# multiplefish/VPLines-SLAM

Hardware: AMD Instinct MI355X
Metric: sliding-window BA solves/sec (10 KF, 200 pts + 80 lines, 5 iters) (higher is better)
Workload: dtype f64

## Files before the change

### vplines-slam_amd/csrc/ba_common.h

```cpp
#pragma once
#include <hip/hip_runtime.h>
#include "ba_types.h"
#include "vpl_math.h"

namespace vpl {

#ifdef VPL_STAMPS
#define VPL_STAMP(B, w, i) do { if (threadIdx.x == 0) (B).dbg[(size_t)(w) * 64 + (i)] = (long long)__builtin_readcyclecounter(); } while (0)
#else
#define VPL_STAMP(B, w, i) do {} while (0)
#endif

__device__ __forceinline__ void count_active(const DevBatch& B, int k) {
  if (B.act && threadIdx.x == 0 && B.launch < ACT_SLOTS) atomicAdd(&B.act[4 * B.launch + k], 1);
}

__device__ __forceinline__ int ordered_window(const DevBatch& B) {
  const int w = B.ord_it == 0 ? (int)blockIdx.x : B.order[(size_t)(B.ord_it & 1) * B.nW + blockIdx.x];
  return __builtin_amdgcn_readfirstlane(w);
}

__device__ __forceinline__ double wave_sum(double v) {
#pragma unroll
  for (int o = 32; o > 0; o >>= 1) v += __shfl_xor(v, o, 64);
// ... 129 lines not shown
  diag_tile_step<8>(d, m, r4, cc, ncol, pivc, bad);  diag_tile_step<9>(d, m, r4, cc, ncol, pivc, bad);
  diag_tile_step<10>(d, m, r4, cc, ncol, pivc, bad); diag_tile_step<11>(d, m, r4, cc, ncol, pivc, bad);
  diag_tile_step<12>(d, m, r4, cc, ncol, pivc, bad); diag_tile_step<13>(d, m, r4, cc, ncol, pivc, bad);
  diag_tile_step<14>(d, m, r4, cc, ncol, pivc, bad); diag_tile_step<15>(d, m, r4, cc, ncol, pivc, bad);
}


__device__ __forceinline__ bool wave_chol16(double* A, int n, int ld, double* Xinv, int lane) {
  const int r4 = lane >> 4, cc = lane & 15;
  double d[4], m[4];
#pragma unroll
  for (int v = 0; v < 4; ++v) {
    const int r = r4 + 4 * v;
    d[v] = (r < n && cc < n) ? A[r * ld + cc] : (r == cc ? 1.0 : 0.0);
    m[v] = r == cc ? 1.0 : 0.0;
  }
  double pivc = 1.0;
  bool bad = false;
  diag_tile_factor(d, m, r4, cc, 16, pivc, bad);
  if (bad) return false;
  const double sq = sqrt(pivc), isq = 1.0 / sq;
#pragma unroll
  for (int v = 0; v < 4; ++v) {
    const int r = r4 + 4 * v;
    const double ir = __shfl(isq, r, 64);
    if (r < n && cc < n) {
      A[r * ld + cc] = r > cc ? d[v] / sq : (r == cc ? sq : 0.0);
      if (Xinv) Xinv[r * ld + cc] = r >= cc ? m[v] * ir : 0.0;
    }
  }
  return true;
}

}
```

### vplines-slam_amd/csrc/ba_ctx.h

```cpp
#pragma once
#include <functional>
#include <map>
#include <string>

#include "vplines_ba.h"
#include "ba_types.h"
#include "ba_stage.h"

struct vpl_ctx {
  int device = 0;
  hipStream_t stream = nullptr;
  DevBatch B;
  std::vector<void*> allocs;
  std::vector<size_t> alloc_bytes;
  bool guards = false;
  std::string err;
  int maxW = 0, maxP = 0, maxPO = 0, maxL = 0, maxLO = 0;
  int nW = 0;
  vpl_ba_options opt;
  bool upload_open = false;
  std::vector<int> h_nP, h_nL;
  std::vector<std::vector<int>> h_lmap;
  std::vector<int> h_mg_m;
  std::vector<int> h_mg_n;
  std::vector<int> h_mg_nb;
  std::vector<int> h_passthrough;
  std::vector<vpl_prior> h_pass_priors;
  bool any_second_new = false;
  int maxPriorN = 0;
  bool prior_resident = false;
  int prior_resident_nW = 0;
  std::vector<int> layout_key;
  bool layout_valid = false;
  bool force_general = false;
  bool schur_mostly_wide = false;
  bool schur_never_wide = false;
  bool schur_wide_all = false;
  bool step_fused = true;
  size_t marg_smem = 0;
  int marg_nmax = 0;
  bool marg_small = false;
  int prior_rule = VPL_PRIOR_PIVOTED_CHOLESKY;
  hipGraphExec_t graph_exec = nullptr;
  bool use_graph = true;
  bool timing = false;
  std::map<std::string, std::pair<double, int>> ktimes;
  std::vector<std::pair<const char*, double>> ltimes;
  int* d_act = nullptr;
  std::vector<std::string> kname_store;
  bool leg_timing = false;
  hipEvent_t leg_ev[6] = {nullptr, nullptr, nullptr, nullptr, nullptr, nullptr};
  double odo_ms[3] = {0, 0, 0};
  std::function<int()> pending;
  Stage stage;
  size_t last_upload_bytes = 0;
  struct vpl_odo* odo = nullptr;
};

static void drop_graph(vpl_ctx* c) {
  if (c->graph_exec) { (void)hipGraphExecDestroy(c->graph_exec); c->graph_exec = nullptr; }
}

static int settle(vpl_ctx* c) {
  if (!c || !c->pending) return VPL_OK;
  std::function<int()> fin;
  fin.swap(c->pending);
  return fin();
}
static int finish_or_defer(vpl_ctx* c, bool async, std::function<int()> fin) {
  if (!async) return fin();
// ... 34 lines not shown
```

### vplines-slam_amd/csrc/ba_lin.h

```cpp
#pragma once
#include "ba_common.h"

namespace vpl {

typedef double v4d_lin __attribute__((ext_vector_type(4)));
constexpr int LIN_THREADS = 512;
constexpr int STG_LD = 17;
constexpr int LIN_STAGE = 8 * 32 * STG_LD;
constexpr int PRE_LDS = 62;
constexpr int LIN_HW = 720;
constexpr int PREP_NMAX = 112;
__host__ __device__ constexpr int lin_stage_doubles(int maxL) {
  const int ln = 8 * LIN_HW + 38 * maxL;
  const int pt = LIN_STAGE + 78 * 36 + NV;
  const int m = ln > pt ? ln : pt;
  return m > 4650 + 3570 ? m : 4650 + 3570;
}
constexpr int PREP_THREADS = 640;
inline size_t prep_smem(int max_prior_n) {
  const int ns = max_prior_n < PREP_NMAX ? max_prior_n : PREP_NMAX;
  return (size_t)((PREP_THREADS / 64) * 675 + ns * ns) * sizeof(double);
}
constexpr size_t PREP_SMEM = (size_t)((PREP_THREADS / 64) * 675 + PREP_NMAX * PREP_NMAX) * sizeof(double);

__device__ __forceinline__ void prep_body(const DevBatch& B, const int w, double* psm, int nstage) {
  const int tid = threadIdx.x;
  const int lane = tid & 63, wv = tid >> 6;
  const int NWV = blockDim.x >> 6;
  double* wsc = psm + wv * 675;
  double* Jl = psm + NWV * 675;
  const int n = B.pr_n[w];
  const bool fits = n > 0 && n <= nstage;
  if (fits) {
    const double* J0g = B.pr_J0 + (size_t)w * B.prS;
    for (int idx = tid; idx < n * n; idx += blockDim.x) Jl[idx] = J0g[idx];
  }
  for (int j = 1 + wv; j < NF; j += NWV) {
    DevPreint& P = B.pre[(size_t)w * NF + j];
    double* G = wsc;
    double* X = wsc + 225;
    double* Pm = wsc + 450;
    for (int k = lane; k < 225; k += 64) G[k] = P.cov[k];
    __builtin_amdgcn_wave_barrier();
    wave_chol16(G, 15, 15, X, lane);
    __builtin_amdgcn_wave_barrier();
    for (int e = lane; e < 225; e += 64) {
      const int a = e / 15, b2 = e % 15;
      double s2 = 0;
      for (int k = (a > b2 ? a : b2); k < 15; ++k) s2 += X[k * 15 + a] * X[k * 15 + b2];
      Pm[e] = s2;
    }
    __builtin_amdgcn_wave_barrier();
    wave_chol16(Pm, 15, 15, nullptr, lane);
    __builtin_amdgcn_wave_barrier();
    for (int e = lane; e < 225; e += 64) {
      const int i = e / 15, jj = e % 15;
      P.sqrt_info[e] = (jj >= i) ? Pm[jj * 15 + i] : 0.0;
    }
    __builtin_amdgcn_wave_barrier();
  }
  if (tid < NF + 1) {
    double* x = tid < NF ? B.pose + ((size_t)w * NF + tid) * 7 : B.ex + (size_t)w * 7;
    Q4 q = mat2q(qmat(qnormalized(qpose(x))));
    if (tid == 0) {
      M3 R0 = qmat(qnormalized(qpose(x)));
      V3 ypr = R2ypr(R0);
      double* g = B.gauge + (size_t)w * 4;
      g[0] = ypr.x; g[1] = x[0]; g[2] = x[1]; g[3] = x[2];
      const double* fr = B.fail_ref + (size_t)w * 13;
      if (fr[0] != 0.0) {
        M3 Rl;
        for (int k = 0; k < 9; ++k) Rl.m[k] = fr[4 + k];
        g[0] = R2ypr(Rl).x; g[1] = fr[1]; g[2] = fr[2]; g[3] = fr[3];
      }
    }
    x[3] = q.x; x[4] = q.y; x[5] = q.z; x[6] = q.w;
    double* xq = psm + 7 * tid;
    xq[0] = x[0]; xq[1] = x[1]; xq[2] = x[2]; xq[3] = q.x; xq[4] = q.y; xq[5] = q.z; xq[6] = q.w;
  }
  __syncthreads();
  const int nL = B.orth_in[w] ? 0 : B.nL[w];
  for (int l = tid; l < nL; l += blockDim.x) {
    const int s = B.ln_start[(size_t)w * B.maxL + l];
    const double* ps = psm + 7 * s;
    const double* ex = psm + 7 * NF;
    M3 Rs = qmat(qpose(ps)), ric = qmat(qpose(ex));
    V3 P{ps[0], ps[1], ps[2]}, tic{ex[0], ex[1], ex[2]};
    V3 twc = P + mul(Rs, tic);
    M3 Rwc = mul(Rs, ric);
    const double* pl = B.plk + ((size_t)w * B.maxL + l) * 6;
    Plk Lc{V3{pl[0], pl[1], pl[2]}, V3{pl[3], pl[4], pl[5]}};
    Plk Lw = plk_to_pose(Lc, Rwc, twc);
    plk_to_orth(Lw, B.orth + ((size_t)w * B.maxL + l) * 4);
  }
  for (int l = tid; l < B.nL[w]; l += blockDim.x) {
    const size_t li = (size_t)w * B.maxL + l;
    const Plk Lw = orth_to_plk(B.orth + li * 4);
    double* o = B.lw + li * 6;
    o[0] = Lw.n.x; o[1] = Lw.n.y; o[2] = Lw.n.z; o[3] = Lw.v.x; o[4] = Lw.v.y; o[5] = Lw.v.z;
  }
  if (n > 0) {
    const double* J0 = B.pr_J0 + (size_t)w * B.prS;
    double* H = B.pr_H + (size_t)w * B.prS;
    const double* Js = fits ? Jl : J0;
    if (fits) {
      const int NT = (n + 15) >> 4, NLT = NT * (NT + 1) / 2, KS = (n + 3) >> 2;
      const int m = lane & 15, kk = lane >> 4;
      for (int t = wv; t < NLT; t += NWV) {
        int ta, tb;
        tri_decode(t, ta, tb);
        const int ca = 16 * ta + m, cb = 16 * tb + m;
        v4d_lin acc = {0, 0, 0, 0};
        for (int ks = 0; ks < KS; ++ks) {
          const int k = 4 * ks + kk;
          const double av = (k < n && ca < n) ? Js[k * n + ca] : 0.0;
          const double bv = (k < n && cb < n) ? Js[k * n + cb] : 0.0;
          acc = __builtin_amdgcn_mfma_f64_16x16x4f64(av, bv, acc, 0, 0, 0);
        }
        const double vals[4] = {acc.x, acc.y, acc.z, acc.w};
#pragma unroll
        for (int v = 0; v < 4; ++v) {
          const int r = 16 * ta + kk + 4 * v, c2 = cb;
          if (r < n && c2 < n && (ta != tb || r >= c2)) {
            H[(size_t)r * n + c2] = vals[v];
            H[(size_t)c2 * n + r] = vals[v];
          }
        }
      }
    } else
    for (int idx = tid; idx < n * n; idx += blockDim.x) {
      int a = idx / n, b = idx % n;
      double s = 0;
      for (int k = 0; k < n; ++k) s += Js[(size_t)k * n + a] * Js[(size_t)k * n + b];
      H[idx] = s;
    }
    for (int c2 = tid; c2 < n; c2 += blockDim.x) {
      double s = 0;
      const double* r0g = B.pr_r0 + (size_t)w * MAXPN;
#pragma unroll 8
      for (int k = 0; k < n; ++k) s += Js[(size_t)k * n + c2] * r0g[k];
      B.pr_g0[(size_t)w * MAXPN + c2] = s;
    }
    if (tid < B.pr_nb[w]) {
      int kind = B.pr_kind[(size_t)w * MAXPB + tid], fr = B.pr_frame[(size_t)w * MAXPB + tid];
      int idx = B.pr_idx[(size_t)w * MAXPB + tid];
      int base = kind == 0 ? 15 * fr : kind == 1 ? 15 * fr + 6 : 165;
      int ls = kind == 1 ? 9 : 6;
      for (int k = 0; k < ls; ++k) B.pr_map[(size_t)w * MAXPN + idx + k] = base + k;
    }
  }
  if (tid == 0) {
    TrState t;
    t.radius = 1e4; t.mu = 1e-8; t.x_cost = 0; t.cand_cost = 0; t.model_cost_change = 0; t.x_norm = 0;
    t.step_norm = 0; t.dogleg_step_norm = 0; t.alpha = 0; t.a1 = t.a2 = t.a3 = 0; t.initial_cost = 0;
    t.iter = 0; t.status = 0; t.reuse = 0; t.step_valid = 0; t.fresh_lin = 0; t.num_successful = 0; t.num_invalid = 0;
    t.pad = 0;
    B.tr[w] = t;
  }
}
__global__ __launch_bounds__(PREP_THREADS) void k_prep(DevBatch B, int nstage) {
  extern __shared__ double psm[];
  prep_body(B, blockIdx.x, psm, nstage);
}

constexpr int HV_DOUBLES = 78 * 36;
constexpr int LIN_PART = 78 * 36 + 72 + 8;
__host__ __device__ __forceinline__ int hvi(int r, int c) {
  const int br = r / 6, bc = c / 6;
  return 36 * (br * (br + 1) / 2 + bc) + 6 * (r - 6 * br) + (c - 6 * bc);
}

inline void lin_asm_entry(int r, int c, int* out) {
  int hv = 0, im = 0;
  const int vr = cam2vis(r), vc = cam2vis(c);
  if (vr >= 0 && vc >= 0) hv = hvi(vr, vc) + 1;
  if (r < 165) {
    const int fr = r / 15, ar = r - 15 * fr, fc = c / 15, bc = c - 15 * fc;
    if (fc == fr) im = 120 * fr + ar * (ar + 1) / 2 + bc + 1;
    else if (fc == fr - 1) im = 11 * 120 + 225 * (fr - 1) + 15 * ar + bc + 1;
  }
  out[0] = hv | im << 16;
  out[1] = r | c << 8;
}

template <int MODE, int ROLE>
__device__ __forceinline__ void lin_body(const DevBatch& B, const int w, double* sm) {
  constexpr bool MARG = MODE != 0;
  constexpr bool PRIOR_ONLY = MODE == 2;
  constexpr bool DO_PTS = ROLE != 2, DO_REST = ROLE != 1;
  static_assert(ROLE == 0 || MODE == 0, "the marginalisation passes are one work-group");
  const int tid = threadIdx.x, T = LIN_THREADS;
  TrState* tr = &B.tr[w];
  if (!MARG) {
    if (tr->status != 0 || tr->fresh_lin) return;
    if (DO_REST) count_active(B, 0);
  }
  if (PRIOR_ONLY && B.mg_n[w] == 0) return;
  double* Hv = sm;
  double* gv = Hv + HV_DOUBLES;
  double* xp = gv + NV;
  double* xs = xp + 84;
  double* imuJ = xs + 99;
  double* imur = imuJ + 4500;
  const int stg_doubles = lin_stage_doubles(B.maxL);
  double* prr = imuJ + stg_doubles;
  double* prdx = prr + MAXPN;
  double* prg = prdx + MAXPN;
  double* red = prg + MAXPN;
  const int PST = B.maxP | 1;
  double* pacc = red + 18;
  double* prH = pacc + 14 * PST;
  const int PRH_N = B.prhN;
  double* plds = prH + PRH_N * (PRH_N + 1) / 2;
  int* invmap = (int*)(plds + 10 * PRE_LDS);
// ... 473 lines not shown
  VPL_STAMP(B, w, 25);
  for (int i = tid; i < 4650; i += T) imuJ[i] = 0.0;
  double sa[2][4];
#pragma unroll
  for (int q = 0; q < 2; ++q) {
    const int f = (tid >> 6) + 8 * q;
    const double* S = B.pre[(size_t)w * NF + (f < 10 ? f : 0) + 1].sqrt_info;
#pragma unroll
    for (int ks = 0; ks < 4; ++ks) {
      const int k = 4 * ks + (lane >> 4), i = lane & 15;
      sa[q][ks] = (f < 10 && i < 15 && k < 15 && k >= i) ? S[i * 15 + k] : 0.0;
    }
  }
  __syncthreads();
  if ((tid & 63) < 10 && tid < 128) {
    const int f = tid & 63, j = f + 1;
    const DevPreint& dp = *(const DevPreint*)(plds + PRE_LDS * f);
    bool act = MARG ? (j == 1 && dp.sum_dt < 10.0) : !(dp.sum_dt > 10.0);
    if (PRIOR_ONLY) act = false;
    if (tid < 64) imuact[f] = act ? 1 : 0;
    if (act) {
      PreInt p = load_preint(dp);
      if (tid < 64) {
        imu_residual_raw(p, xp + 7 * (j - 1), xs + 9 * (j - 1), xp + 7 * j, xs + 9 * j, B.opt.g_norm, imur + 15 * f);
      } else {
        ImuJac JB = imu_jacobian_raw(p, xp + 7 * (j - 1), xs + 9 * (j - 1), xp + 7 * j, xs + 9 * j, B.opt.g_norm);
        imu_jac_dense(JB, imuJ + 450 * f);
      }
    }
  }
  __syncthreads();
  VPL_STAMP(B, w, 28);
  constexpr int ASM_PER_THREAD = (NCP + LIN_THREADS - 1) / LIN_THREADS;
  int2 asmd[ASM_PER_THREAD];
#pragma unroll
  for (int u = 0; u < ASM_PER_THREAD; ++u) {
    const int e = u * T + tid;
    asmd[u] = ((const int2*)B.asm_tab)[e < NCP ? e : 0];
  }
  double* imuH = imuJ + 4650;
  {
    const int wvi = tid >> 6, m16 = lane & 15, kk = lane >> 4;
    v4d_lin cd[2] = {{0, 0, 0, 0}, {0, 0, 0, 0}};
    for (int i = tid; i < 120; i += T) imuH[i] = 0.0;
#pragma unroll
    for (int q = 0; q < 2; ++q) {
      const int f = wvi + 8 * q;
      if (f >= 10) break;
      double* J = imuJ + 450 * f;
      double* rr = imur + 15 * f;
      const bool on = imuact[f] != 0;
      v4d_lin jw[2] = {{0, 0, 0, 0}, {0, 0, 0, 0}};
#pragma unroll
      for (int ct = 0; ct < 2; ++ct) {
        const int c = 16 * ct + m16;
#pragma unroll
        for (int ks = 0; ks < 4; ++ks) {
          const int k = 4 * ks + kk;
          const double bv = k < 15 ? (c < 30 ? J[k * 30 + c] : (c == 30 ? rr[k] : 0.0)) : 0.0;
          jw[ct] = __builtin_amdgcn_mfma_f64_16x16x4f64(on ? sa[q][ks] : 0.0, bv, jw[ct], 0, 0, 0);
        }
      }
      __builtin_amdgcn_wave_barrier();
      if (on) {
#pragma unroll
        for (int ct = 0; ct < 2; ++ct) {
          const double vals[4] = {jw[ct].x, jw[ct].y, jw[ct].z, jw[ct].w};
          const int c = 16 * ct + m16;
#pragma unroll
          for (int v = 0; v < 4; ++v) {
            const int r = kk + 4 * v;
// ... 48 lines not shown
#pragma unroll
      for (int v = 0; v < 4; ++v) {
        const int i0 = kk + 4 * v, j0 = m16;
        if (i0 < 15 && j0 <= i0) imuH[120 * f + i0 * (i0 + 1) / 2 + j0] += keep[v];
      }
    }
  }
  __syncthreads();
  if (tid < 10 && imuact[tid]) {
    double s = 0;
    for (int k = 0; k < 15; ++k) s += imur[15 * tid + k] * imur[15 * tid + k];
    cost += 0.5 * s;
  }


  if (ROLE == 2) {
    if (tid == 0) {
      while (__hip_atomic_load(&B.lin_flag[w], __ATOMIC_RELAXED, __HIP_MEMORY_SCOPE_AGENT) != 1) __builtin_amdgcn_s_sleep(32);
      __hip_atomic_store(&B.lin_flag[w], 0, __ATOMIC_RELAXED, __HIP_MEMORY_SCOPE_AGENT);
    }
    __syncthreads();
    const double* part = B.lin_part + (size_t)w * LIN_PART;
    for (int i = tid; i < HV_DOUBLES + NV; i += T) sm[i] += __hip_atomic_load(&part[i], __ATOMIC_RELAXED, __HIP_MEMORY_SCOPE_AGENT);
    if (tid == 0) cost += __hip_atomic_load(&part[HV_DOUBLES + NV], __ATOMIC_RELAXED, __HIP_MEMORY_SCOPE_AGENT);
    __syncthreads();
  } else if (!MARG) {
    if (tid == 0) cost += cost_pts;
  }
  VPL_STAMP(B, w, 20);
  double* Hout = B.Hcc + (size_t)w * NCP;
  const double* pH = B.pr_H + (size_t)w * B.prS;
  VPL_STAMP(B, w, 26);
  const bool prior_lds = n > 0 && n <= PRH_N;
  {
#pragma unroll
    for (int u = 0; u < ASM_PER_THREAD; ++u) {
      const int e = u * T + tid;
      if (e >= NCP) continue;
      const int hv = asmd[u].x & 0xffff, im = asmd[u].x >> 16, r = asmd[u].y & 255, c = asmd[u].y >> 8;
      const double vh = Hv[hv ? hv - 1 : 0], vi = imuH[im ? im - 1 : 0];
      const int ir = prior_lds ? invmap[r] : -1, ic = prior_lds ? invmap[c] : -1;
      const bool hp = ir >= 0 && ic >= 0;
      const int hi_ = ic > ir ? ic : ir, lo_ = ic > ir ? ir : ic;
      const double vp = prH[hp ? hi_ * (hi_ + 1) / 2 + lo_ : 0];
      double v = hv ? vh : 0.0;
      v += im ? vi : 0.0;
      v += hp ? vp : 0.0;
      if (!ex_free && r >= 165) v = 0.0;
      Hout[e] = v;
    }
  }
  VPL_STAMP(B, w, 27);
  if (n > PRH_N) {
    __syncthreads();
    const int np = n * (n + 1) / 2;
    for (int base = 0; base < np; base += 4 * T) {
      double ph[4];
      int tr_[4], tc_[4];
#pragma unroll
      for (int u = 0; u < 4; ++u) {
        const int e = base + u * T + tid;
        ph[u] = 0.0; tr_[u] = -1; tc_[u] = 0;
        if (e < np) {
          int i, j;
          tri_decode(e, i, j);
          ph[u] = pH[(size_t)i * n + j];
          const int ri = B.pr_map[(size_t)w * MAXPN + i], rj = B.pr_map[(size_t)w * MAXPN + j];
          tr_[u] = ri > rj ? ri : rj;
          tc_[u] = ri > rj ? rj : ri;
        }
      }
#pragma unroll
      for (int u = 0; u < 4; ++u)
        if (tr_[u] >= 0 && (ex_free || tr_[u] < 165)) Hout[(size_t)tr_[u] * (tr_[u] + 1) / 2 + tc_[u]] += ph[u];
    }
  }
  for (int r = tid; r < NC; r += T) {
    double v = 0.0;
    const int vr = cam2vis(r);
    if (vr >= 0) v += gv[vr];
    if (r < 165) {
      const int fr = r / 15;
      if (fr >= 1 && imuact[fr - 1]) {
        const double* J = imuJ + 450 * (fr - 1);
        const double* rr = imur + 15 * (fr - 1);
        const int a = r - 15 * (fr - 1);
// ... 68 lines not shown
```

### vplines-slam_amd/csrc/ba_marg.h

```cpp
#pragma once
#include "ba_common.h"

namespace vpl {

__device__ __forceinline__ void gauge_body(const DevBatch& B, const int w) {
  const int tid = threadIdx.x;
  __shared__ double rd[9], p0a[3], p0b[3], newpose[NF * 7], newex[7];
  const double* gz = B.gauge + (size_t)w * 4;
  double* pose = B.pose + (size_t)w * 77;
  double* sb = B.sb + (size_t)w * 99;
  double* ex = B.ex + (size_t)w * 7;
  if (tid == 0) {
    V3 ypr00 = R2ypr(qmat(qpose(pose)));
    double y_diff = gz[0] - ypr00.x;
    M3 R = ypr2R(V3{y_diff, 0, 0});
    for (int k = 0; k < 9; ++k) rd[k] = R.m[k];
    for (int k = 0; k < 3; ++k) { p0a[k] = pose[k]; p0b[k] = gz[1 + k]; }
  }
  __syncthreads();
  M3 rot_diff;
  for (int k = 0; k < 9; ++k) rot_diff.m[k] = rd[k];
  V3 P0a{p0a[0], p0a[1], p0a[2]}, P0b{p0b[0], p0b[1], p0b[2]};
  if (tid < NF) {
    const double* x = pose + 7 * tid;
// ... 456 lines not shown
  const int fixed = L.EB + L.nd * L.ldd + 16 * 17 + L.nd + (L.nd * 16 < 640 ? 640 : L.nd * 16) + nn + 16 + 24 + (nn + L.nd + 2 * L.loff + 16) / 2 + 4;
  L.mtrows = MTROWS_MAX;
  while (L.mtrows > 32 && (size_t)(fixed + L.mtrows * 74) * sizeof(double) > (small ? MARG_LDS_SMALL : MARG_LDS_BIG)) L.mtrows -= 32;
  L.total = fixed + L.mtrows * 74;
  return L;
}

template <int T>
__device__ __forceinline__ void marg_body(const DevBatch& B, const int w, double* sm) {
  const int tid = threadIdx.x;
  const int nP = B.nP[w], nL = B.nL[w];
  const int nb = B.mg_nb[w];
  const int n = B.mg_n[w];
  if (n == 0) return;
  const bool second_new = B.opt.marginalization_flag == 1;
  const int md = second_new ? 6 : 15;
  const MargLayout L = marg_layout(n, T == 256);
  const int nd = md + n, ldd = L.ldd, ldm = L.ldm;
  double* G = sm;
  double* Ad = G + L.EB;
  const int MTROWS = L.mtrows;
  double* tile = Ad + nd * ldd;
  double* E15 = tile + MTROWS * 74;
  double* bv = E15 + 16 * 17;
  double* tmp = bv + nd;
  double* lam = tmp + (nd * 16 < 640 ? 640 : nd * 16);
  double* red = lam + (n < 2 ? 2 : n) + 16;
  int* perm = (int*)(red + 24);
  int* dmap = perm + (n < 16 ? 16 : n) + (n & 1);
  int* lst = dmap + nd + (nd & 1);
  const int LOFF = L.loff;
  __shared__ int s_np0, s_nl0, s_flag[4], s_phase[4];

  if (tid < md) dmap[tid] = second_new ? 15 * (NF - 2) + tid : (tid < 9 ? 6 + tid : tid - 9);
  if (tid < nb) {
    const int kind = B.mg_kind[(size_t)w * MAXPB + tid];
    const int base = B.mg_cam[(size_t)w * MAXPB + tid], idx = B.mg_idx[(size_t)w * MAXPB + tid];
    const int ls = kind == 1 ? 9 : 6;
    for (int k = 0; k < ls; ++k) dmap[md + idx + k] = base + k;
  }
  if (tid >= 64 && !second_new) {
    const int np0 = min(LOFF, B.ps_cnt[(size_t)w * (NF + 1) + 1]);
    for (int a = tid - 64; a < np0; a += T - 64) lst[a] = B.ps_list[(size_t)w * B.maxP + a];
    if (tid == 64) s_np0 = np0;
  }
  if (tid < 64) {
    int c = 0;
    if (!second_new)
      for (int l0 = 0; l0 < nL; l0 += 64) {
        const int l = l0 + tid;
        const bool on = l < nL && B.ln_start[(size_t)w * B.maxL + l] == 0 && B.ln_nobs[(size_t)w * B.maxL + l] >= 2 &&
                        !B.ln_removed[(size_t)w * B.maxL + l];
        const unsigned long long m = __ballot(on);
        if (on && c + __popcll(m & ((1ull << tid) - 1ull)) < LOFF) lst[LOFF + c + __popcll(m & ((1ull << tid) - 1ull))] = l;
        c += __popcll(m);
      }
    if (tid == 0) { s_nl0 = min(c, LOFF); if (second_new) s_np0 = 0; }
  }
  __syncthreads();
  VPL_STAMP(B, w, 32);
  const double* Hcc = B.Hcc + (size_t)w * NCP;
  const double* gc = B.gc + (size_t)w * NC;
  for (int base = 0; base < nd * nd; base += 8 * T) {
    double hv[8];
    int dst[8];
#pragma unroll
    for (int u = 0; u < 8; ++u) {
      const int it = base + u * T + tid;
      dst[u] = -1;
      hv[u] = 0.0;
      if (it < nd * nd) {
        const int i = it / nd, j = it - i * nd;
        const int ci = dmap[i], cj = dmap[j];
        dst[u] = i * ldd + j;
        hv[u] = ci >= cj ? Hcc[tri(ci, cj)] : Hcc[tri(cj, ci)];
      }
    }
#pragma unroll
    for (int u = 0; u < 8; ++u)
      if (dst[u] >= 0) Ad[dst[u]] = hv[u];
  }
  VPL_STAMP(B, w, 38);
  for (int i = tid; i < nd; i += T) bv[i] = gc[dmap[i]];
  int* vlist = (int*)tmp;
  int* vinv = vlist + 96;
  if (tid < 64) {
    const int lane = tid;
    const bool f0 = lane < nd && cam2vis(dmap[lane]) >= 0;
    const bool f1 = lane + 64 < nd && cam2vis(dmap[lane + 64]) >= 0;
    const unsigned long long m0 = __ballot(f0), m1 = __ballot(f1);
    const unsigned long long below = (1ull << lane) - 1ull;
    if (f0) vlist[__popcll(m0 & below)] = lane;
    if (f1) vlist[__popcll(m0) + __popcll(m1 & below)] = lane + 64;
    if (lane == 0) s_flag[2] = __popcll(m0) + __popcll(m1);
  } else if (tid < 64 + 72) {
// ... 299 lines not shown
```

### vplines-slam_amd/csrc/ba_types.h

```cpp
#pragma once
#include <stdint.h>

namespace vpl {

constexpr int NF = 11;
constexpr int NC = 171;
constexpr int NV = 72;
__host__ __device__ inline int wcol(int c, int s, int WS) {
  if (c >= 66) return WS - 72 + c;
  const int cc = c - 6 * s;
  return (cc >= 0 && cc < WS - 6) ? cc : -1;
}
constexpr int NCP = NC * (NC + 1) / 2;
constexpr int MAXPB = 23;
constexpr int MAXPN = 171;
constexpr int ACT_SLOTS = 64;
constexpr int SK_WSTRIDE = 64;
constexpr int NZ_N = 2628 + 1089 + 1890 + 540;
constexpr int SACC_N = 74 * 75 / 2;
constexpr int MAXKEEP = 80;

__host__ __device__ inline int vis2cam(int v) { return v < 66 ? 15 * (v / 6) + (v % 6) : 165 + (v - 66); }
__host__ __device__ inline int tri(int r, int c) { return r * (r + 1) / 2 + c; }

struct DevOptions {
  int num_iterations, estimate_extrinsic, marginalization_flag, remove_line_outliers;
  double sqrt_info_point, sqrt_info_line, sqrt_info_vp, g_norm, huber_delta;
};

struct DevPreint {
  double sum_dt;
  double dp[3], dq[4] , dv[3], lba[3], lbg[3];
  double dp_dba[9], dp_dbg[9], dq_dbg[9], dv_dba[9], dv_dbg[9];
  double cov[225];
  double sqrt_info[225];
};

struct TrState {
  double radius, mu, x_cost, cand_cost, model_cost_change, x_norm, step_norm, dogleg_step_norm;
  double alpha, a1 , a2 , a3 , initial_cost;
  int iter;
  int status;
  int reuse;
  int step_valid;
  int fresh_lin;
  int num_successful, num_invalid;
  int pad;
};

struct DevBatch {
  int nW;
  int maxP, maxPO, maxL, maxLO;
  int nfull;
// ... 36 lines not shown
  double *pr_H;
  double *pr_g0;
  int prS;
  int *pr_map;

  double *Hcc, *gc;
  int *asm_tab;
  double *Hpp, *gp, *Wp;
  double *Hll, *gl, *Wl;
  int WS, wfill;
  int *order;
  int *ord_cnt;
  int ord_it;
  double *lchol;

  int *sk_tab, *sk_wave;
  int maxKS;
  double *sacc;
  double *ycs;
  double *sx;
  int *path;
  int step_fused;
  int *nz_tab;

  TrState *tr;
  double *scale, *diag, *grad, *gn;

  int *mg_n, *mg_nb;
  int *mg_kind, *mg_frame, *mg_idx, *mg_cam;
  double *mg_x0;
  double *mg_J0, *mg_r0;
  double *mg_A, *mg_b;
  int *mg_m;
  long long *dbg;
  int *act;
  int launch;
};


struct KeepSrc {
  int nP; const int *pt_start, *pt_nobs;
  int nL; const int *ln_start, *ln_nobs, *ln_removed;
  int pr_nb; const int *pr_kind, *pr_frame;
  bool imu01;
};

__host__ __device__ inline void keep_tables_old(const KeepSrc& S, int* kind, int* frame, int* idx, int* cam, int* n_out,
                                                int* nb_out, int* m_out) {
  bool pose_t[NF], sb_t[NF];
  for (int f = 0; f < NF; ++f) { pose_t[f] = false; sb_t[f] = false; }
  bool ex_t = false, frame0 = false;
  int m = 0;
  for (int p = 0; p < S.nP; ++p)
    if (S.pt_start[p] == 0) { for (int k = 1; k < S.pt_nobs[p]; ++k) pose_t[k] = true; ex_t = frame0 = true; m += 1; }
  for (int l = 0; l < S.nL; ++l)
    if (S.ln_start[l] == 0 && S.ln_nobs[l] >= 2 && !(S.ln_removed && S.ln_removed[l])) {
      for (int k = 1; k < S.ln_nobs[l]; ++k) pose_t[k] = true;
      ex_t = frame0 = true; m += 4;
    }
  for (int b = 0; b < S.pr_nb; ++b) {
    if (S.pr_kind[b] == 0) pose_t[S.pr_frame[b]] = true;
    else if (S.pr_kind[b] == 1) sb_t[S.pr_frame[b]] = true;
    else ex_t = true;
  }
  if (S.imu01) { pose_t[0] = pose_t[1] = true; sb_t[0] = sb_t[1] = true; }
  int nb = 0, n = 0;
// ... 32 lines not shown
```

### vplines-slam_amd/csrc/ba_upload.h

```cpp
#pragma once
#include "ba_ctx.h"
#include "ba_odo.h"
#include "ba_pack.h"
#include "host_common.h"

static void to_dev_preint(const vpl_preintegration& p, DevPreint& d) {
  d.sum_dt = p.sum_dt;
  for (int k = 0; k < 3; ++k) { d.dp[k] = p.delta_p[k]; d.dv[k] = p.delta_v[k]; d.lba[k] = p.linearized_ba[k]; d.lbg[k] = p.linearized_bg[k]; }
  for (int k = 0; k < 4; ++k) d.dq[k] = p.delta_q[k];
  auto blk = [&](double* o, int r0, int c0) {
    for (int i = 0; i < 3; ++i)
      for (int j = 0; j < 3; ++j) o[3 * i + j] = p.jacobian[(r0 + i) * 15 + c0 + j];
  };
  blk(d.dp_dba, 0, 9); blk(d.dp_dbg, 0, 12); blk(d.dq_dbg, 3, 12); blk(d.dv_dba, 6, 9); blk(d.dv_dbg, 6, 12);
  std::memcpy(d.cov, p.covariance, sizeof(d.cov));
  std::memset(d.sqrt_info, 0, sizeof(d.sqrt_info));
}

struct UploadArena {
  Span<double> pose, sb, ex, invd, plk, pt_obs, ln_obs, fail_ref, orth, pr_x0, pr_r0;
  Span<int> nP, nL, pt_start, pt_nobs, pt_off, ln_start, ln_nobs, ln_off, ln_tri, pu_cnt, pu_cnt0, sk_tab, sk_wave, path, nLO, lo_ln,
      ll_tab, ll_np, ps_list, ps_cnt, orth_in, pr_n, pr_nb, pr_kind, pr_frame, pr_idx, mg_n, mg_nb, mg_kind, mg_frame, mg_idx, mg_cam, mg_m;
  Span<DevPreint> pre;
  std::vector<Span<double>> J0;
// ... 467 lines not shown
  if (!same_layout) pack_units(SG, A, W, B.maxPR, lane.get(), sub.get());
  std::memcpy(A.mg_m.p, c->h_mg_m.data(), W * 4);
  c->h_mg_n.assign(A.mg_n.begin(), A.mg_n.end());
  c->h_mg_nb.assign(A.mg_nb.begin(), A.mg_nb.end());
  if (odo)
    for (size_t w = 0; w < W; ++w)
      A.odo_marg[w] = (opt->marginalization_flag != VPL_MARGIN_NONE && c->h_passthrough[w] < 0) ? 1 + A.mg_nb[w] : 0;
  if (!same_layout) c->schur_mostly_wide = schur_total_w > 0 && 20 * schur_wide_w > 7 * schur_total_w;
  if (c->force_general) std::fill(A.path.begin(), A.path.end(), 1);
  if (SG.overflow) return fail(c, VPL_E_CAPACITY, "internal: staging arena bound too small");
  stage_upload(SG, A, B, W, same_layout, dev_prior, odo);
  if (chained && (rc = hand_over_priors(c, ctab, prev_prS))) return rc;
  HIPCHK(c, stage_run(c->stage, c->stream, true, &c->last_upload_bytes));
  if (odo) {
    hipLaunchKernelGGL(k_odo_gather, dim3(nW), dim3(ODO_THREADS), 0, c->stream, B, odo->store, (const int*)odo->d_psrc, (const int*)odo->d_lsrc);
    if (odo->tab) hipLaunchKernelGGL(k_odo_prior_load, dim3(nW), dim3(ODO_THREADS), 0, c->stream, B, odo->prior, (const int*)odo->d_has);
    HIPCHK(c, hipGetLastError());
  }
  if (c->leg_timing) HIPCHK(c, hipEventRecord(c->leg_ev[1], c->stream));
  HIPCHK(c, hipStreamSynchronize(c->stream));
  c->layout_valid = true;
  return VPL_OK;
}
static int upload_impl(vpl_ctx* c, int nW, const vpl_window* win, const vpl_ba_options* opt, bool all_lines, bool chained = false,
                       const OdoSrc* odo = nullptr) {
  const int rc = upload_body(c, nW, win, opt, all_lines, chained, odo);
  if (c) {
    if (rc != VPL_OK && c->upload_open) { c->nW = 0; c->prior_resident = false; }
    c->upload_open = false;
  }
  return rc;
}

static int restore_states(vpl_ctx* c, bool plk) {
  const DevBatch& B = c->B;
  const size_t W = c->nW;
  HIPCHK(c, hipMemcpyAsync(B.pose, B.pose_0, W * 77 * 8, hipMemcpyDeviceToDevice, c->stream));
  HIPCHK(c, hipMemcpyAsync(B.sb, B.sb_0, W * 99 * 8, hipMemcpyDeviceToDevice, c->stream));
  HIPCHK(c, hipMemcpyAsync(B.ex, B.ex_0, W * 7 * 8, hipMemcpyDeviceToDevice, c->stream));
  HIPCHK(c, hipMemcpyAsync(B.invd, B.invd_0, W * B.maxP * 8, hipMemcpyDeviceToDevice, c->stream));
  if (plk) HIPCHK(c, hipMemcpyAsync(B.plk, B.plk_0, W * B.maxL * 6 * 8, hipMemcpyDeviceToDevice, c->stream));
  return VPL_OK;
}
```

### vplines-slam_amd/csrc/vplines_ba.hip

```cpp
#include <hip/hip_runtime.h>

#include <algorithm>
#include <chrono>
#include <memory>
#include <cstdlib>
#include <cstring>
#include <string>
#include <vector>

#include "vplines_ba.h"
#include "ba_types.h"
#include "ba_lin.h"
#include "ba_pack.h"
#include "ba_solve.h"
#include "ba_step.h"
#include "ba_marg.h"
#include "ba_prior_eig.h"
#include "ba_lineopt.h"
#include "ba_factors.h"
#include "ba_odo.h"
#include "odo_tracks.h"
#include "host_common.h"

using namespace vpl;
// ... 85 lines not shown
    B.ncu = ncu;
  }
  B.maxPR = max_point_unit_rounds(B.maxP, B.maxPO);
  B.maxKS = max_schur_ksteps(B.maxP, B.maxL);
  B.llSlots = line_lane_slots(B.maxL);
  const size_t W = max_windows;
  hipError_t e = hipSuccess;
#define AL(ptr, n) if (e == hipSuccess) e = dalloc(c, &B.ptr, (size_t)(n))
  AL(pose, W * 77); AL(sb, W * 99); AL(ex, W * 7); AL(invd, W * B.maxP); AL(orth, W * B.maxL * 4);
  AL(pose_c, W * 77); AL(sb_c, W * 99); AL(ex_c, W * 7); AL(invd_c, W * B.maxP); AL(orth_c, W * B.maxL * 4); AL(lw, W * B.maxL * 6); AL(lw_c, W * B.maxL * 6);
  AL(lin_part, W * LIN_PART); AL(lin_pcost, W); AL(lin_flag, W);
  AL(pose_0, W * 77); AL(sb_0, W * 99); AL(ex_0, W * 7); AL(invd_0, W * B.maxP); AL(plk_0, W * B.maxL * 6);
  AL(plk, W * B.maxL * 6); AL(gauge, W * 4); AL(fail_ref, W * 13); AL(orth_in, W);
  AL(nP, W); AL(nL, W);
  AL(pt_start, W * B.maxP); AL(pt_nobs, W * B.maxP); AL(pt_off, W * B.maxP); AL(pt_obs, W * B.maxPO * 3);
  AL(ps_list, W * B.maxP); AL(ps_cnt, W * (NF + 1)); AL(pu_lane, W * B.maxPR * 1024); AL(pu_sub, W * B.maxPR * 512); AL(pu_cnt, W); AL(pu_cnt0, W);
  AL(ln_start, W * B.maxL); AL(ln_nobs, W * B.maxL); AL(ln_off, W * B.maxL); AL(ln_obs, W * B.maxLO * 8);
  AL(nLO, W); AL(lo_ln, W * B.maxLO);
  AL(ll_tab, W * B.llSlots * 2); AL(ll_np, W);
  AL(pre, W * NF);
  AL(pr_n, W); AL(pr_nb, W); AL(pr_kind, W * MAXPB); AL(pr_frame, W * MAXPB); AL(pr_idx, W * MAXPB);
  AL(pr_x0, W * MAXPB * 9); AL(pr_J0, W * MAXPN * MAXPN); AL(pr_r0, W * MAXPN); AL(pr_H, W * MAXPN * MAXPN); AL(pr_g0, W * MAXPN);
  AL(pr_map, W * MAXPN);
  AL(Hcc, W * NCP); AL(gc, W * NC); AL(asm_tab, 2 * NCP); AL(Hpp, W * B.maxP); AL(gp, W * B.maxP); AL(Wp, W * B.maxP * NV);
  AL(Hll, W * B.maxL * 16); AL(gl, W * B.maxL * 4); AL(Wl, W * B.maxL * 4 * NV); AL(lchol, W * B.maxL * 10);
  AL(tr, W);
  AL(scale, W * B.nfull); AL(diag, W * B.nfull); AL(grad, W * B.nfull); AL(gn, W * B.nfull);
  AL(mg_n, W); AL(mg_nb, W); AL(mg_kind, W * MAXPB); AL(mg_frame, W * MAXPB); AL(mg_idx, W * MAXPB);
  AL(mg_cam, W * MAXPB); AL(mg_x0, W * MAXPB * 9); AL(mg_J0, W * MAXKEEP * MAXKEEP); AL(mg_r0, W * MAXKEEP);
  AL(mg_A, W * MAXKEEP * MAXKEEP); AL(mg_b, W * MAXKEEP); AL(mg_m, W); AL(dbg, W * 64); AL(ln_removed, W * B.maxL); AL(ln_tri, W * B.maxL);
  if (e == hipSuccess) e = dalloc(c, &c->d_act, (size_t)ACT_SLOTS * 4);
  AL(order, 2 * W); AL(ord_cnt, 4);
  AL(sk_tab, W * B.maxKS * 4); AL(sk_wave, W * 8 * SK_WSTRIDE); AL(sacc, W * SACC_N); AL(nz_tab, NZ_N); AL(ycs, W * 176); AL(sx, W * 8); AL(path, W);
#undef AL
  if (e != hipSuccess) return VPL_E_HIP;
  if (lin_smem_base(c->maxP, c->maxL) > LIN_LDS_BUDGET) return VPL_E_CAPACITY;
  B.prhN = lin_prh_n(c->maxP, c->maxL);
  {
    std::vector<int> tab(2 * NCP);
    for (int r = 0, e2 = 0; r < NC; ++r)
      for (int cc = 0; cc <= r; ++cc, ++e2) lin_asm_entry(r, cc, &tab[2 * e2]);
    if (hipMemcpy(B.asm_tab, tab.data(), tab.size() * sizeof(int), hipMemcpyHostToDevice) != hipSuccess) return VPL_E_HIP;
  }
  {
    std::vector<int> nz;
    for (int r = 0; r < NC; ++r)
      for (int cc = 0; cc <= r; ++cc) {
        const bool vis = cam2vis(r) >= 0 && cam2vis(cc) >= 0;
        const int fr = r < 165 ? r / 15 : -1, fc = cc < 165 ? cc / 15 : -1;
        const bool band = fr >= 0 && fc >= 0 && (fr == fc || fr == fc + 1);
        const bool sb0 = cc >= 6 && cc < 15 && cam2vis(r) >= 0;
        if (vis || band || sb0) nz.push_back(tri(r, cc) | r << 14 | cc << 22);
      }
    if ((int)nz.size() != NZ_N || hipMemcpy(B.nz_tab, nz.data(), nz.size() * sizeof(int), hipMemcpyHostToDevice) != hipSuccess) return VPL_E_HIP;
  }
  static size_t lin_max = 0, solve_max = 0, schur_max = 0, back_max = 0, step_max = 0;
  lin_max = std::max(lin_max, lin_smem(c->maxP, c->maxL));
  solve_max = std::max(solve_max, solve_smem(c->maxP, c->maxL));
  schur_max = std::max(schur_max, schur_smem(c->maxP, c->maxL));
  back_max = std::max(back_max, back_smem(c->maxP, c->maxL));
  step_max = std::max(step_max, step_smem(c->maxP, c->maxL));
  if (schur_max > 159 * 1024 || back_max > 159 * 1024) return VPL_E_CAPACITY;
  const std::pair<const void*, size_t> lds[] = {
      {(const void*)k_lin2, lin_max}, {(const void*)k_lin<1>, lin_max}, {(const void*)k_lin<2>, lin_max},
      {(const void*)k_solve, solve_max}, {(const void*)k_schur<3>, schur_max}, {(const void*)k_schur<5>, schur_max},
      {(const void*)k_schur_mixed, schur_max}, {(const void*)k_chol, CHOL_SMEM}, {(const void*)k_back, back_max},
      {(const void*)k_step<3, false>, step_max}, {(const void*)k_step<3, true>, step_max}, {(const void*)k_step<5, false>, step_max},
      {(const void*)k_prep, PREP_SMEM}, {(const void*)k_marg<MARG_THREADS>, 159 * 1024}, {(const void*)k_marg<256>, MARG_LDS_SMALL},
      {(const void*)k_prior_eigen, prior_eig_layout(MAXKEEP).bytes}};
  for (const auto& k : lds)
    if (hipFuncSetAttribute(k.first, hipFuncAttributeMaxDynamicSharedMemorySize, (int)k.second) != hipSuccess) return VPL_E_HIP;
  vpl_ba_default_options(&c->opt);
  if (const char* gv = std::getenv("VPL_BA_GRAPH")) c->use_graph = std::atoi(gv) != 0;
  if (const char* gv = std::getenv("VPL_BA_GENERAL")) c->force_general = std::atoi(gv) != 0;
  if (const char* gv = std::getenv("VPL_BA_STEP_FUSED")) c->step_fused = std::atoi(gv) != 0;
  if (const char* gv = std::getenv("VPL_BA_SCHUR_WIDE")) { c->schur_wide_all = std::atoi(gv) > 0; c->schur_never_wide = std::atoi(gv) < 0; }
  return VPL_OK;
}

int vpl_ctx_create(vpl_ctx** out, int device, int max_windows, int max_points, int max_point_obs, int max_lines,
                   int max_line_obs) {
  if (!out || max_windows < 1 || max_points < 0 || max_lines < 0) return VPL_E_INVALID;
  int ndev = 0;
  if (hipGetDeviceCount(&ndev) != hipSuccess || ndev == 0 || device >= ndev) return VPL_E_NODEVICE;
  if (hipSetDevice(device) != hipSuccess) return VPL_E_NODEVICE;
  vpl_ctx* c = new vpl_ctx();
  const int rc = ctx_init(c, device, max_windows, max_points, max_point_obs, max_lines, max_line_obs);
  if (rc != VPL_OK) {
    free_arrays(c);
    delete c;
    return rc;
  }
  *out = c;
  return VPL_OK;
}

void vpl_ctx_destroy(vpl_ctx* c) {
  if (!c) return;
  (void)hipSetDevice(c->device);
  (void)hipDeviceSynchronize();
  drop_graph(c);
  free_arrays(c);
  c->stage.release();
  for (hipEvent_t& e : c->leg_ev) if (e) (void)hipEventDestroy(e);
  delete c;
}

int vpl_ctx_set_stream(vpl_ctx* c, void* s) {
// ... 818 lines not shown
```

Measured before the change: 263,000.

## Build dense marginalization block in linearize, fuse state restore into one kernel

In the marginalization linearize pass, the dense marginalization Hessian block is now gathered directly into a new per-window buffer mg_D via a dense index map. k_marg then copies it contiguously instead of gathering from the packed Hcc, and the packed assembly is skipped unless VPL_BA_MARG_PACKED is set. The five device-to-device state restore memcpys are replaced by one segmented copy kernel, which cuts launch overhead. k_prep threads are halved with a min-blocks launch bound, and timing stamps are added. The new path adds a global buffer and does an O(nd^2) scattered read per window.

```diff
diff --git a/vplines-slam_amd/csrc/ba_common.h b/vplines-slam_amd/csrc/ba_common.h
--- a/vplines-slam_amd/csrc/ba_common.h
+++ b/vplines-slam_amd/csrc/ba_common.h
@@ -185,4 +185,18 @@
   return true;
 }
 
-}
+__device__ __forceinline__ int marg_dense_map(const DevBatch& B, const int w, int* dmap) {
+  const int tid = threadIdx.x;
+  const bool second_new = B.opt.marginalization_flag == 1;
+  const int md = second_new ? 6 : 15;
+  if (tid < md) dmap[tid] = second_new ? 15 * (NF - 2) + tid : (tid < 9 ? 6 + tid : tid - 9);
+  if (tid < B.mg_nb[w]) {
+    const int kind = B.mg_kind[(size_t)w * MAXPB + tid];
+    const int base = B.mg_cam[(size_t)w * MAXPB + tid], idx = B.mg_idx[(size_t)w * MAXPB + tid];
+    const int ls = kind == 1 ? 9 : 6;
+    for (int k = 0; k < ls; ++k) dmap[md + idx + k] = base + k;
+  }
+  return md;
+}
+
+}
diff --git a/vplines-slam_amd/csrc/ba_ctx.h b/vplines-slam_amd/csrc/ba_ctx.h
--- a/vplines-slam_amd/csrc/ba_ctx.h
+++ b/vplines-slam_amd/csrc/ba_ctx.h
@@ -36,6 +36,7 @@
   bool schur_mostly_wide = false;
   bool schur_never_wide = false;
   bool schur_wide_all = false;
+  bool marg_packed = false;
   bool step_fused = true;
   size_t marg_smem = 0;
   int marg_nmax = 0;
diff --git a/vplines-slam_amd/csrc/ba_lin.h b/vplines-slam_amd/csrc/ba_lin.h
--- a/vplines-slam_amd/csrc/ba_lin.h
+++ b/vplines-slam_amd/csrc/ba_lin.h
@@ -16,7 +16,7 @@
   const int m = ln > pt ? ln : pt;
   return m > 4650 + 3570 ? m : 4650 + 3570;
 }
-constexpr int PREP_THREADS = 640;
+constexpr int PREP_THREADS = 320;
 inline size_t prep_smem(int max_prior_n) {
   const int ns = max_prior_n < PREP_NMAX ? max_prior_n : PREP_NMAX;
   return (size_t)((PREP_THREADS / 64) * 675 + ns * ns) * sizeof(double);
@@ -35,6 +35,7 @@
     const double* J0g = B.pr_J0 + (size_t)w * B.prS;
     for (int idx = tid; idx < n * n; idx += blockDim.x) Jl[idx] = J0g[idx];
   }
+  VPL_STAMP(B, w, 14);
   for (int j = 1 + wv; j < NF; j += NWV) {
     DevPreint& P = B.pre[(size_t)w * NF + j];
     double* G = wsc;
@@ -59,6 +60,7 @@
     }
     __builtin_amdgcn_wave_barrier();
   }
+  VPL_STAMP(B, w, 15);
   if (tid < NF + 1) {
     double* x = tid < NF ? B.pose + ((size_t)w * NF + tid) * 7 : B.ex + (size_t)w * 7;
     Q4 q = mat2q(qmat(qnormalized(qpose(x))));
@@ -99,6 +101,7 @@
     double* o = B.lw + li * 6;
     o[0] = Lw.n.x; o[1] = Lw.n.y; o[2] = Lw.n.z; o[3] = Lw.v.x; o[4] = Lw.v.y; o[5] = Lw.v.z;
   }
+  VPL_STAMP(B, w, 17);
   if (n > 0) {
     const double* J0 = B.pr_J0 + (size_t)w * B.prS;
     double* H = B.pr_H + (size_t)w * B.prS;
@@ -149,6 +152,7 @@
       for (int k = 0; k < ls; ++k) B.pr_map[(size_t)w * MAXPN + idx + k] = base + k;
     }
   }
+  VPL_STAMP(B, w, 19);
   if (tid == 0) {
     TrState t;
     t.radius = 1e4; t.mu = 1e-8; t.x_cost = 0; t.cand_cost = 0; t.model_cost_change = 0; t.x_norm = 0;
@@ -158,7 +162,7 @@
     B.tr[w] = t;
   }
 }
-__global__ __launch_bounds__(PREP_THREADS) void k_prep(DevBatch B, int nstage) {
+__global__ __launch_bounds__(PREP_THREADS, 3) void k_prep(DevBatch B, int nstage) {
   extern __shared__ double psm[];
   prep_body(B, blockIdx.x, psm, nstage);
 }
@@ -170,7 +174,7 @@
   return 36 * (br * (br + 1) / 2 + bc) + 6 * (r - 6 * br) + (c - 6 * bc);
 }
 
-inline void lin_asm_entry(int r, int c, int* out) {
+__host__ __device__ inline int lin_asm_src(int r, int c) {
   int hv = 0, im = 0;
   const int vr = cam2vis(r), vc = cam2vis(c);
   if (vr >= 0 && vc >= 0) hv = hvi(vr, vc) + 1;
@@ -179,7 +183,10 @@
     if (fc == fr) im = 120 * fr + ar * (ar + 1) / 2 + bc + 1;
     else if (fc == fr - 1) im = 11 * 120 + 225 * (fr - 1) + 15 * ar + bc + 1;
   }
-  out[0] = hv | im << 16;
+  return hv | im << 16;
+}
+inline void lin_asm_entry(int r, int c, int* out) {
+  out[0] = lin_asm_src(r, c);
   out[1] = r | c << 8;
 }
 
@@ -719,11 +726,12 @@
   __syncthreads();
   VPL_STAMP(B, w, 28);
   constexpr int ASM_PER_THREAD = (NCP + LIN_THREADS - 1) / LIN_THREADS;
+  const bool packed = !MARG || B.marg_packed;
   int2 asmd[ASM_PER_THREAD];
 #pragma unroll
   for (int u = 0; u < ASM_PER_THREAD; ++u) {
     const int e = u * T + tid;
-    asmd[u] = ((const int2*)B.asm_tab)[e < NCP ? e : 0];
+    asmd[u] = packed ? ((const int2*)B.asm_tab)[e < NCP ? e : 0] : int2{0, 0};
   }
   double* imuH = imuJ + 4650;
   {
@@ -838,7 +846,7 @@
   const double* pH = B.pr_H + (size_t)w * B.prS;
   VPL_STAMP(B, w, 26);
   const bool prior_lds = n > 0 && n <= PRH_N;
-  {
+  if (packed) {
 #pragma unroll
     for (int u = 0; u < ASM_PER_THREAD; ++u) {
       const int e = u * T + tid;
@@ -855,9 +863,32 @@
       if (!ex_free && r >= 165) v = 0.0;
       Hout[e] = v;
     }
+  } else if constexpr (MARG) {
+    int* dmap = (int*)plds;
+    const int nd = marg_dense_map(B, w, dmap) + B.mg_n[w];
+    __syncthreads();
+    double* D = B.mg_D + (size_t)w * MARG_ND * MARG_ND;
+    const bool prior_hbm = n > PRH_N;
+    for (int it = tid; it < nd * nd && nd <= MARG_ND; it += T) {
+      const int i = it / nd, j = it - i * nd;
+      const int di = dmap[i], dj = dmap[j];
+      const int r = di > dj ? di : dj, c = di > dj ? dj : di;
+      const int src = lin_asm_src(r, c);
+      const int hv = src & 0xffff, im = src >> 16;
+      const double vh = Hv[hv ? hv - 1 : 0], vi = imuH[im ? im - 1 : 0];
+      const int pr_ = n > 0 ? invmap[r] : -1, pc_ = n > 0 ? invmap[c] : -1;
+      const int hi_ = pc_ > pr_ ? pc_ : pr_, lo_ = pc_ > pr_ ? pr_ : pc_;
+      const bool hp = prior_lds && lo_ >= 0;
+      const double vp = prH[hp ? hi_ * (hi_ + 1) / 2 + lo_ : 0];
+      double v = hv ? vh : 0.0;
+      v += im ? vi : 0.0;
+      v += hp ? vp : 0.0;
+      if (prior_hbm && lo_ >= 0) v += pH[(size_t)hi_ * n + lo_];
+      D[it] = v;
+    }
   }
   VPL_STAMP(B, w, 27);
-  if (n > PRH_N) {
+  if (packed && n > PRH_N) {
     __syncthreads();
     const int np = n * (n + 1) / 2;
     for (int base = 0; base < np; base += 4 * T) {
diff --git a/vplines-slam_amd/csrc/ba_marg.h b/vplines-slam_amd/csrc/ba_marg.h
--- a/vplines-slam_amd/csrc/ba_marg.h
+++ b/vplines-slam_amd/csrc/ba_marg.h
@@ -512,13 +512,7 @@
   const int LOFF = L.loff;
   __shared__ int s_np0, s_nl0, s_flag[4], s_phase[4];
 
-  if (tid < md) dmap[tid] = second_new ? 15 * (NF - 2) + tid : (tid < 9 ? 6 + tid : tid - 9);
-  if (tid < nb) {
-    const int kind = B.mg_kind[(size_t)w * MAXPB + tid];
-    const int base = B.mg_cam[(size_t)w * MAXPB + tid], idx = B.mg_idx[(size_t)w * MAXPB + tid];
-    const int ls = kind == 1 ? 9 : 6;
-    for (int k = 0; k < ls; ++k) dmap[md + idx + k] = base + k;
-  }
+  marg_dense_map(B, w, dmap);
   if (tid >= 64 && !second_new) {
     const int np0 = min(LOFF, B.ps_cnt[(size_t)w * (NF + 1) + 1]);
     for (int a = tid - 64; a < np0; a += T - 64) lst[a] = B.ps_list[(size_t)w * B.maxP + a];
@@ -541,6 +535,22 @@
   VPL_STAMP(B, w, 32);
   const double* Hcc = B.Hcc + (size_t)w * NCP;
   const double* gc = B.gc + (size_t)w * NC;
+  if (!B.marg_packed) {
+    const double* D = B.mg_D + (size_t)w * MARG_ND * MARG_ND;
+    for (int base = 0; base < nd * nd; base += 8 * T) {
+      double hv[8];
+#pragma unroll
+      for (int u = 0; u < 8; ++u) {
+        const int it = base + u * T + tid;
+        hv[u] = it < nd * nd ? D[it] : 0.0;
+      }
+#pragma unroll
+      for (int u = 0; u < 8; ++u) {
+        const int it = base + u * T + tid;
+        if (it < nd * nd) { const int i = it / nd; Ad[i * ldd + (it - i * nd)] = hv[u]; }
+      }
+    }
+  } else
   for (int base = 0; base < nd * nd; base += 8 * T) {
     double hv[8];
     int dst[8];
diff --git a/vplines-slam_amd/csrc/ba_types.h b/vplines-slam_amd/csrc/ba_types.h
--- a/vplines-slam_amd/csrc/ba_types.h
+++ b/vplines-slam_amd/csrc/ba_types.h
@@ -19,6 +19,7 @@
 constexpr int NZ_N = 2628 + 1089 + 1890 + 540;
 constexpr int SACC_N = 74 * 75 / 2;
 constexpr int MAXKEEP = 80;
+constexpr int MARG_ND = 15 + MAXKEEP;
 
 __host__ __device__ inline int vis2cam(int v) { return v < 66 ? 15 * (v / 6) + (v % 6) : 165 + (v - 66); }
 __host__ __device__ inline int tri(int r, int c) { return r * (r + 1) / 2 + c; }
@@ -121,6 +122,8 @@
   double *mg_J0, *mg_r0;
   double *mg_A, *mg_b;
   int *mg_m;
+  double *mg_D;
+  int marg_packed;
   long long *dbg;
   int *act;
   int launch;
diff --git a/vplines-slam_amd/csrc/ba_upload.h b/vplines-slam_amd/csrc/ba_upload.h
--- a/vplines-slam_amd/csrc/ba_upload.h
+++ b/vplines-slam_amd/csrc/ba_upload.h
@@ -523,13 +523,39 @@
   return rc;
 }
 
+struct RestoreSegs {
+  double* dst[5];
+  const double* src[5];
+  unsigned end[5];
+};
+__global__ __launch_bounds__(256) void k_restore_states(const RestoreSegs R, const int nseg) {
+  const unsigned total = R.end[nseg - 1];
+  for (unsigned i = blockIdx.x * 256u + threadIdx.x; i < total; i += gridDim.x * 256u) {
+    int k = 0;
+    while (i >= R.end[k]) ++k;
+    const unsigned off = i - (k ? R.end[k - 1] : 0u);
+    R.dst[k][off] = R.src[k][off];
+  }
+}
 static int restore_states(vpl_ctx* c, bool plk) {
   const DevBatch& B = c->B;
   const size_t W = c->nW;
-  HIPCHK(c, hipMemcpyAsync(B.pose, B.pose_0, W * 77 * 8, hipMemcpyDeviceToDevice, c->stream));
-  HIPCHK(c, hipMemcpyAsync(B.sb, B.sb_0, W * 99 * 8, hipMemcpyDeviceToDevice, c->stream));
-  HIPCHK(c, hipMemcpyAsync(B.ex, B.ex_0, W * 7 * 8, hipMemcpyDeviceToDevice, c->stream));
-  HIPCHK(c, hipMemcpyAsync(B.invd, B.invd_0, W * B.maxP * 8, hipMemcpyDeviceToDevice, c->stream));
-  if (plk) HIPCHK(c, hipMemcpyAsync(B.plk, B.plk_0, W * B.maxL * 6 * 8, hipMemcpyDeviceToDevice, c->stream));
-  return VPL_OK;
-}
+  RestoreSegs R{};
+  const size_t cnt[5] = {W * 77, W * 99, W * 7, W * B.maxP, W * B.maxL * 6};
+  double* const dst[5] = {B.pose, B.sb, B.ex, B.invd, B.plk};
+  const double* const src[5] = {B.pose_0, B.sb_0, B.ex_0, B.invd_0, B.plk_0};
+  int nseg = 0;
+  size_t total = 0;
+  for (int k = 0; k < (plk ? 5 : 4); ++k) {
+    if (cnt[k] == 0) continue;
+    total += cnt[k];
+    R.dst[nseg] = dst[k]; R.src[nseg] = src[k]; R.end[nseg] = (unsigned)total;
+    ++nseg;
+  }
+  if (total > 0xffffffffu) return fail(c, VPL_E_CAPACITY, "internal: batch states too large for one restore launch");
+  if (nseg == 0) return VPL_OK;
+  const unsigned blocks = (unsigned)std::min<size_t>((total + 255) / 256, 2048);
+  hipLaunchKernelGGL(k_restore_states, dim3(blocks), dim3(256), 0, c->stream, R, nseg);
+  HIPCHK(c, hipGetLastError());
+  return VPL_OK;
+}
diff --git a/vplines-slam_amd/csrc/vplines_ba.hip b/vplines-slam_amd/csrc/vplines_ba.hip
--- a/vplines-slam_amd/csrc/vplines_ba.hip
+++ b/vplines-slam_amd/csrc/vplines_ba.hip
@@ -141,6 +141,7 @@
   if (e == hipSuccess) e = dalloc(c, &c->d_act, (size_t)ACT_SLOTS * 4);
   AL(order, 2 * W); AL(ord_cnt, 4);
   AL(sk_tab, W * B.maxKS * 4); AL(sk_wave, W * 8 * SK_WSTRIDE); AL(sacc, W * SACC_N); AL(nz_tab, NZ_N); AL(ycs, W * 176); AL(sx, W * 8); AL(path, W);
+  AL(mg_D, W * MARG_ND * MARG_ND);
 #undef AL
   if (e != hipSuccess) return VPL_E_HIP;
   if (lin_smem_base(c->maxP, c->maxL) > LIN_LDS_BUDGET) return VPL_E_CAPACITY;
@@ -183,6 +184,8 @@
   if (const char* gv = std::getenv("VPL_BA_GRAPH")) c->use_graph = std::atoi(gv) != 0;
   if (const char* gv = std::getenv("VPL_BA_GENERAL")) c->force_general = std::atoi(gv) != 0;
   if (const char* gv = std::getenv("VPL_BA_STEP_FUSED")) c->step_fused = std::atoi(gv) != 0;
+  if (const char* gv = std::getenv("VPL_BA_MARG_PACKED")) c->marg_packed = std::atoi(gv) != 0;
+  B.marg_packed = c->marg_packed;
   if (const char* gv = std::getenv("VPL_BA_SCHUR_WIDE")) { c->schur_wide_all = std::atoi(gv) > 0; c->schur_never_wide = std::atoi(gv) < 0; }
   return VPL_OK;
 }
```

Measured after the change: 264,200 (median of 3 runs). No clear change (+0.5%).
